# alanqrwang/nwhead

Measured on AMD Instinct MI355X. Metric: query-predictions/sec, higher is better.
Workload: dtype f32; 1 GPU; K3 predict('full'): B=256 queries/step vs bank N=50000 d=512 C=200, bank sharded 1-way, 26 query batches coalesced per launch; B=256, N_support=50000, d=512, C=200, parallelism=support-shard x1

## Files before the change

include/nwhead_hip.h:

```cpp
#ifndef NWHEAD_HIP_H
#define NWHEAD_HIP_H

#include <stddef.h>
#include <stdint.h>

#ifdef __cplusplus
extern "C" {
#endif

#define NW_ABI_VERSION 2

typedef enum {
    NW_SCORE_EUCLIDEAN = 0,
    NW_SCORE_HYPERSPHERE = 1,
    NW_SCORE_COSINE = 2,
    NW_SCORE_DOT = 3,
    NW_SCORE_CLIP = 4
} nw_score_kind;

typedef enum {
    NW_OK = 0,
    NW_ERR_INVALID_ARG = -1,
    NW_ERR_UNSUPPORTED = -2,
    NW_ERR_WORKSPACE = -3,
    NW_ERR_LAUNCH = -4,
    NW_ERR_NO_DEVICE = -5
} nw_status;

int nw_abi_version(void);
const char *nw_status_string(int status);
int nw_device_check(void);

int nw_scores_f32(const float *q, const float *s, float *scores,
                  int64_t B, int64_t N, int64_t d,
                  int kind, const float *logit_scale_dev, int sup_batched, void *stream);

int nw_row_norm2_f32(const float *x, float *n2, int64_t rows, int64_t d, void *stream);

int nw_split_rows_f16x2(const float *x, float *out_split, float *row_scale, float *row_norm2,
                        int64_t rows, int64_t d, void *stream);

typedef struct nw_fwd_opts {
    uint32_t struct_size;
    int32_t persistent_wgs;
    int32_t force_split;
    int32_t reserved;
    const void *tables;
    size_t tables_bytes;
    const int64_t *tables_sy;
    int64_t tables_N;
} nw_fwd_opts;

size_t nw_fwd_workspace_bytes(int64_t B, int64_t N, int64_t d, int64_t C);
int nw_fwd_f32(const float *q, const float *s, const int64_t *sy, const float *s_norm2,
               const float *s_split, const float *s_scale,
               float *out, float *scores_out, float *lse_out, float *weights_out,
               void *workspace, size_t workspace_bytes,
               int64_t B, int64_t N, int64_t d, int64_t C,
               int kind, const float *logit_scale_dev,
               int sup_batched, int labels_batched, const nw_fwd_opts *opts, void *stream);

int nw_fwd_partial_f32(const float *q, const float *s, const int64_t *sy, const float *s_norm2,
                       const float *s_split, const float *s_scale,
                       float *m, float *den, float *num,
                       void *workspace, size_t workspace_bytes,
                       int64_t B, int64_t N, int64_t d, int64_t C,
                       int kind, const float *logit_scale_dev, const nw_fwd_opts *opts, void *stream);
int nw_merge_finalize_f32(const float *m, const float *den, const float *num, float *out,
                          int64_t G, int64_t B, int64_t C,
                          int64_t stride_m, int64_t stride_den, int64_t stride_num,
                          const int64_t *class_lo, int64_t C_local, void *stream);

size_t nw_bank_tables_bytes(int64_t N);
int nw_bank_tables_build(const int64_t *sy, int64_t N, int64_t C, void *tables, size_t tables_bytes, void *stream);


size_t nw_bwd_workspace_bytes(int64_t B, int64_t N, int64_t d, int64_t C, int kind, int sup_batched);
int nw_bwd_f32(const float *q, const float *s, const int64_t *sy,
               const float *scores, const float *lse, const float *out, const float *gout,
               float *gq, float *gs, float *glogit_scale,
               void *workspace, size_t workspace_bytes,
               int64_t B, int64_t N, int64_t d, int64_t C,
               int kind, const float *logit_scale_dev,
               int sup_batched, int labels_batched, void *stream);
int nw_bwd_uses_split(int64_t B, int64_t N, int64_t d, int64_t C, int sup_batched);
int nw_bwd_bank_f32(const float *q, const float *s, const float *s_norm2, const float *s_split,
                    const float *s_scale, const int64_t *sy,
                    const float *scores, const float *lse, const float *out, const float *gout,
                    float *gq, float *gs, float *glogit_scale,
                    void *workspace, size_t workspace_bytes,
                    int64_t B, int64_t N, int64_t d, int64_t C,
                    int kind, const float *logit_scale_dev,
                    int sup_batched, int labels_batched, void *stream);


int nw_support_influence_f32(const float *probs, const int64_t *qy, const float *w,
                             const int64_t *sy, float *infl,
// ... 182 lines not shown
```

nwhead_amd/_lib.py:

```python
from __future__ import annotations

import ctypes as C
import os

_HERE = os.path.dirname(os.path.abspath(__file__))
LIB_PATH = os.environ.get("NW_HIP_LIB") or os.path.join(_HERE, "csrc", "libnwhead_hip.so")

SCORE_KINDS = {"euclidean": 0, "hypersphere_euclidean": 1, "cosine": 2, "dotproduct": 3, "clip": 4}

_p = C.c_void_p
_i64 = C.c_int64
_int = C.c_int
_sz = C.c_size_t

SIGNATURES = {
    "nw_abi_version": (_int, []),
    "nw_status_string": (C.c_char_p, [_int]),
    "nw_device_check": (_int, []),
    "nw_scores_f32": (_int, [_p, _p, _p, _i64, _i64, _i64, _int, _p, _int, _p]),
    "nw_fwd_workspace_bytes": (_sz, [_i64, _i64, _i64, _i64]),
    "nw_row_norm2_f32": (_int, [_p, _p, _i64, _i64, _p]),
    "nw_split_rows_f16x2": (_int, [_p, _p, _p, _p, _i64, _i64, _p]),
    "nw_fwd_f32": (_int, [_p, _p, _p, _p, _p, _p, _p, _p, _p, _p, _p, _sz, _i64, _i64, _i64, _i64, _int, _p, _int, _int, _p, _p]),
    "nw_fwd_partial_f32": (_int, [_p, _p, _p, _p, _p, _p, _p, _p, _p, _p, _sz, _i64, _i64, _i64, _i64, _int, _p, _p, _p]),
    "nw_merge_finalize_f32": (_int, [_p, _p, _p, _p, _i64, _i64, _i64, _i64, _i64, _i64, _p, _i64, _p]),
    "nw_bank_tables_bytes": (_sz, [_i64]),
    "nw_bank_tables_build": (_int, [_p, _i64, _i64, _p, _sz, _p]),
    "nw_bwd_workspace_bytes": (_sz, [_i64, _i64, _i64, _i64, _int, _int]),
    "nw_bwd_f32": (_int, [_p] * 10 + [_p, _sz, _i64, _i64, _i64, _i64, _int, _p, _int, _int, _p]),
    "nw_bwd_uses_split": (_int, [_i64, _i64, _i64, _i64, _int]),
    "nw_bwd_bank_f32": (_int, [_p] * 13 + [_p, _sz, _i64, _i64, _i64, _i64, _int, _p, _int, _int, _p]),
    "nw_support_influence_f32": (_int, [_p, _p, _p, _p, _p, _i64, _i64, _i64, _p]),
    "nw_aggregate_f32": (_int, [_p] * 5 + [_i64, _i64, _i64, _int, _p]),
    "nw_aggregate_bwd_f32": (_int, [_p] * 6 + [_i64, _i64, _i64, _int, _p]),
    "nw_fwd_influence_f32": (_int, [_p] * 11 + [_sz, _i64, _i64, _i64, _i64, _int, _p, _p, _p]),
    "nw_topk_f32": (_int, [_p, _p, _p, _i64, _i64, _i64, _p]),
    "nw_scale_shift_relu_f32": (_int, [_p, _p, _p, _p, _i64, _i64, _i64, _i64, _int, _p]),
    "nw_bias_act_nhwc_f32": (_int, [_p, _p, _p, _int, _p, _i64, _i64, _p]),
    "nw_scale_shift_relu_avgpool2_f32": (_int, [_p, _p, _p, _p, _i64, _i64, _i64, _i64, _i64, _int, _p]),
    "nw_conv3x3_workgroups": (_i64, [_i64, _i64, _i64, _i64, _i64]),
    "nw_conv3x3_workspace_bytes": (_sz, [_i64, _i64, _i64, _i64, _i64]),
    "nw_conv3x3_f32": (_int, [_p, _i64, _p, _p, _p, _i64, _int, _p, _i64, _p, _sz, _i64, _i64, _i64, _i64, _i64, _p]),
    "nw_conv1x1_workspace_bytes": (_sz, [_i64, _i64, _i64, _i64]),
    "nw_conv1x1_f32": (_int, [_p, _i64, _p, _p, _int, _p, _p, _int, _p, _i64, _p, _sz, _i64, _i64, _i64, _i64, _p]),
    "nw_bn_relu_train_fwd_f32": (_int, [_p] * 10 + [_i64, _i64, _i64, _i64, C.c_float, C.c_float, _int, _p]),
    "nw_bn_relu_train_bwd_f32": (_int, [_p] * 12 + [_i64, _i64, _i64, _i64, _i64, _int, _p]),
    "nw_absmax_f32": (_int, [_p, _i64, _p, _p]),
    "nw_to_nhwc_pad_f32": (_int, [_p, _p, _p, _i64, _i64, _i64, _i64, _i64, _i64, _i64, _p]),
    "nw_conv2d_nhwc_supported": (_int, [_i64] * 9),
    "nw_conv2d_nhwc_f16x2": (_int, [_p, _p, _p, _p, _p, _p, _int, _p, _p] + [_i64] * 11 + [_p, _p]),
# ... 64 lines not shown
        raise NWHipError("libnwhead_hip.so ABI version mismatch")
    _lib = lib
    sync_knobs()
    return lib


class WgradJob(C.Structure):
    _fields_ = [("x", C.c_void_p), ("amax_x", C.c_void_p), ("gy", C.c_void_p), ("amax_g", C.c_void_p), ("dw", C.c_void_p)] + \
               [(k, C.c_int64) for k in ("n", "H", "W", "Cin", "Cout", "KH", "KW", "stride", "pad", "ldx", "ldg", "out_oihw")] + \
               [("pre_x", C.c_void_p)] + [(k, C.c_int64) for k in ("rowrun_stride", "in_H", "in_W", "row0", "col0")]


class SgdParam(C.Structure):
    _fields_ = [("param", C.c_void_p), ("grad", C.c_void_p), ("momentum_buf", C.c_void_p), ("n", C.c_int64)]


class ConvBnStat(C.Structure):
    _fields_ = [("x", C.c_void_p), ("ldx", C.c_int64), ("mean", C.c_void_p), ("invstd", C.c_void_p), ("gamma", C.c_void_p),
                ("beta", C.c_void_p), ("partials", C.c_void_p)]


class FwdOpts(C.Structure):
    _fields_ = [("struct_size", C.c_uint32), ("persistent_wgs", C.c_int32), ("force_split", C.c_int32),
                ("reserved", C.c_int32), ("tables", C.c_void_p), ("tables_bytes", C.c_size_t),
                ("tables_sy", C.c_void_p), ("tables_N", C.c_int64)]


KNOBS = ("pvar", "qg", "tile_rs", "merge_mq", "merge_per_query", "merge_no_global_tables", "persistent_any_rs", "no_persistent",
         "split_queries", "bwd_no_mfma", "bwd_split", "coeff_threads", "xgemm_wgs", "xgemm_nbuf", "split_lbits", "conv_gather",
         "conv_max_wgs", "wgrad_min_stages", "conv_skip_cfgs", "wgrad_batch_wgs", "bn_inline_fin", "conv_moments_per_tile",
         "conv_force_cfg")
_KNOB_UNSET = -2 ** 31
_knob_state = {}


def sync_knobs():
    if _lib is None:
        return
    for k in KNOBS:
        v = os.environ.get("NW_" + k.upper())
        val = _KNOB_UNSET if v is None or v == "" else int(v)
        if _knob_state.get(k, _KNOB_UNSET) != val:
            _lib.nw_debug_set(k.encode(), val)
            _knob_state[k] = val


def force_split():
    return os.environ.get("NW_SPLIT_ALWAYS", "") == "1"


def fwd_opts(tables=None, tables_bytes=0, persistent_wgs=0, tables_sy=None, tables_n=-1):
    return FwdOpts(C.sizeof(FwdOpts), int(persistent_wgs), int(force_split()), 0, tables, int(tables_bytes), tables_sy,
                   int(tables_n))


def check(status: int, what: str):
    if status != 0:
        msg = load().nw_status_string(status).decode()
        raise NWHipError(f"{what}: {msg} (status {status})")
```

nwhead_amd/csrc/capi.hip:

```cpp
#include <cstddef>
#include <cstdlib>
#include <string.h>
#include "nw_internal.h"

namespace {
inline size_t align256(size_t x) { return (x + 255) & ~(size_t)255; }
inline bool bad_kind(int kind) { return kind < NW_SCORE_EUCLIDEAN || kind > NW_SCORE_CLIP; }
}

static bool split_pays(int64_t B, int64_t N, int64_t d) {
    return nw::fwd_opts().force_split || (double)B * (double)N * (double)d >= 2.0e8;
}

namespace nw {
namespace {
thread_local FwdOpts tl_fwd_opts;
int g_knobs[KNOB_COUNT];
bool g_knobs_init = [] { for (int& k : g_knobs) k = KNOB_UNSET; return true; }();
const char* const knob_names[KNOB_COUNT] = {
    "pvar", "qg", "tile_rs", "merge_mq", "merge_per_query", "merge_no_global_tables", "persistent_any_rs", "no_persistent",
    "split_queries", "bwd_no_mfma", "bwd_split", "coeff_threads", "xgemm_wgs", "xgemm_nbuf", "split_lbits", "conv_gather",
    "conv_max_wgs", "wgrad_min_stages", "conv_skip_cfgs", "wgrad_batch_wgs", "bn_inline_fin", "conv_moments_per_tile",
    "conv_force_cfg"};
}
const FwdOpts& fwd_opts() { return tl_fwd_opts; }
int knob(int id) { return (id >= 0 && id < KNOB_COUNT) ? __atomic_load_n(&g_knobs[id], __ATOMIC_RELAXED) : KNOB_UNSET; }
}

namespace {
struct OptsGuard {
    nw::FwdOpts saved;
    explicit OptsGuard(const nw_fwd_opts* o) : saved(nw::tl_fwd_opts) {
        nw::FwdOpts f;
        if (o && o->struct_size >= offsetof(nw_fwd_opts, tables)) {
            f.persistent_wgs = o->persistent_wgs;
            f.force_split = o->force_split;
        }
        if (o && o->struct_size >= sizeof(nw_fwd_opts)) {
            f.tables = static_cast<const char*>(o->tables);
            f.tables_bytes = o->tables_bytes;
            f.tables_sy = o->tables_sy;
            f.tables_N = o->tables_N;
        }
        nw::tl_fwd_opts = f;
    }
    ~OptsGuard() { nw::tl_fwd_opts = saved; }
};
}

extern "C" int nw_debug_set(const char* name, int value) {
    if (!name) return NW_ERR_INVALID_ARG;
    for (int k = 0; k < nw::KNOB_COUNT; ++k)
        if (!strcmp(name, nw::knob_names[k])) {
            __atomic_store_n(&nw::g_knobs[k], value, __ATOMIC_RELAXED);
            return NW_OK;
        }
    return NW_ERR_INVALID_ARG;
}

extern "C" int nw_abi_version(void) { return NW_ABI_VERSION; }

extern "C" const char* nw_status_string(int status) {
    switch (status) {
        case NW_OK: return "ok";
        case NW_ERR_INVALID_ARG: return "invalid argument";
// ... 191 lines not shown
```

nwhead_amd/csrc/fused.hip:

```cpp
#include <mutex>
#include <utility>
#include <vector>
#include "fused_impl.h"
#include <cstring>

namespace nw {

#define NW_EXTERN_FUSED_KIND(K)                                                                          \
    extern template int launch_fused_kind<K>(const float*, const float*, const int64_t*, const float*,   \
                                             const float*,                                               \
                                             const float*, float*, float*, float*, float*, float*,       \
                                             float*, void*, size_t, int, int, int, int, hipStream_t);
NW_EXTERN_FUSED_KIND(NW_SCORE_EUCLIDEAN)
NW_EXTERN_FUSED_KIND(NW_SCORE_HYPERSPHERE)
NW_EXTERN_FUSED_KIND(NW_SCORE_COSINE)
NW_EXTERN_FUSED_KIND(NW_SCORE_DOT)
NW_EXTERN_FUSED_KIND(NW_SCORE_CLIP)
#undef NW_EXTERN_FUSED_KIND

namespace {
struct TileTimer {
    bool on = false;
    std::vector<std::pair<hipEvent_t, hipEvent_t>> ev;
    std::vector<std::pair<hipEvent_t, hipEvent_t>> pool;
// ... 67 lines not shown
    for (const auto& m : map)
        if (!strcmp(m.n, name)) return knob(m.k) == 1;
    return false;
}

inline size_t al256(size_t x) { return (x + 255) & ~(size_t)255; }

size_t fused_layout(int64_t B, int64_t n_stiles, int BS, char* base, FusedWs* ws, int64_t C) {
    size_t off = 0;
    auto take = [&](size_t bytes) {
        char* p = base ? base + off : nullptr;
        off += al256(bytes);
        return p;
    };
    FusedWs w;
    w.m = reinterpret_cast<float*>(take((size_t)n_stiles * B * 4));
    w.den = reinterpret_cast<float*>(take((size_t)n_stiles * B * 4));
    w.nrun = reinterpret_cast<int*>(take((size_t)n_stiles * 4));
    w.lab = reinterpret_cast<int*>(take((size_t)n_stiles * BS * 4));
    w.num = reinterpret_cast<float*>(take((size_t)n_stiles * BS * B * 4));
    w.runid = reinterpret_cast<int*>(take(((size_t)n_stiles * BS + 64) * 4));
    w.bnd = reinterpret_cast<int*>(take((size_t)n_stiles * 2 * 4));
    w.ctab = reinterpret_cast<int*>(take((size_t)C * (3 + 4) * 4));
    if (ws) *ws = w;
    return off;
}

namespace {

constexpr int MTHREADS = 512, MENT = 4, MTPT = 16;
template <bool PARTIAL, int MQ, int TMODE>
__global__ __launch_bounds__(MTHREADS) void nw_merge_runs_kernel(
    const float* __restrict__ ws_m, const float* __restrict__ ws_den, const int* __restrict__ ws_nrun,
    const int* __restrict__ ws_lab, const float* __restrict__ ws_num, float* __restrict__ out,
    float* __restrict__ lse, float* __restrict__ m_out, float* __restrict__ den_out,
    float* __restrict__ num_out, int B, int C, int n_stiles, int BS, const int* __restrict__ ctab) {
    constexpr bool TABLES = TMODE != 0;
    constexpr bool LTAB = TMODE == 1;
    constexpr int ML = MTHREADS / MQ;
    constexpr int MNS = MQ + 1;
    constexpr int NW = MTHREADS / 64;
    constexpr float LN2 = 0.693147180559945309417f;
    static_assert(MQ <= 32 && (MQ & (MQ - 1)) == 0, "a wave holds whole groups of MQ queries");
    extern __shared__ __attribute__((aligned(16))) char smem[];
    float* red = reinterpret_cast<float*>(smem);
    float* Ms = red + 2 * NW * MQ;
    float* inv_s = Ms + MQ;
    int* lds_tab = reinterpret_cast<int*>(inv_s + MQ);
    int* cnt = TMODE == 2 ? const_cast<int*>(ctab) : lds_tab;
    int* tlo = cnt + C;
    int* thi = tlo + C;
    int* ent = thi + C;
    float* res = reinterpret_cast<float*>(lds_tab + (size_t)C * (3 + MENT));
    const int tid = threadIdx.x, bq = tid & (MQ - 1), sl = tid / MQ, wave = tid >> 6;
    const int b0 = blockIdx.x * MQ;
    const int b = min(b0 + bq, B - 1);

    const bool in_regs = n_stiles <= ML * MTPT;
    float mr[MTPT], dr[MTPT];
    float M = -INFINITY;
    if (in_regs) {
#pragma unroll
        for (int u = 0; u < MTPT; ++u) {
            const int t = sl + u * ML;
            const bool ok = t < n_stiles;
            mr[u] = ok ? ws_m[(size_t)t * B + b] : -INFINITY;
            dr[u] = ok ? ws_den[(size_t)t * B + b] : 0.f;
        }
    }
    int tnr = 0, tl3[3] = {-1, -1, -1};
    const bool one_pass_tables = LTAB && n_stiles <= MTHREADS;
    if (one_pass_tables && tid < n_stiles) {
        tnr = ws_nrun[tid];
        const int* lt = ws_lab + (size_t)tid * BS;
        tl3[0] = lt[0];
        tl3[1] = lt[1];
        tl3[2] = lt[2];
    }
    if (LTAB) {
        for (int c = tid; c < C; c += MTHREADS) {
            cnt[c] = 0;
            tlo[c] = 0x7fffffff;
            thi[c] = -1;
        }
    }
    if (in_regs) {
#pragma unroll
        for (int u = 0; u < MTPT; ++u) M = fmaxf(M, mr[u]);
    } else {
        for (int t = sl; t < n_stiles; t += ML) M = fmaxf(M, ws_m[(size_t)t * B + b]);
    }
#pragma unroll
    for (int o = 32; o >= MQ; o >>= 1) M = fmaxf(M, __shfl_xor(M, o));
    if ((tid & 63) < MQ) red[wave * MQ + bq] = M;
    __syncthreads();
    if (LTAB) {
        auto add_tile = [&](int t, int nr, const int (&l3)[3]) {
            const int* lt = ws_lab + (size_t)t * BS;
            for (int r = 0; r < nr; ++r) {
                const int y = r < 3 ? l3[r] : lt[r];
                if (y < 0) continue;
                atomicMin(&tlo[y], t);
                atomicMax(&thi[y], t);
                const int slot = atomicAdd(&cnt[y], 1);
                if (slot < MENT) ent[y * MENT + slot] = t * BS + r;
            }
        };
        if (one_pass_tables) {
            if (tid < n_stiles) add_tile(tid, tnr, tl3);
        } else {
            for (int t = tid; t < n_stiles; t += MTHREADS) {
// ... 33 lines not shown
                        if (e[j] < e[j - 1]) { const int x = e[j]; e[j] = e[j - 1]; e[j - 1] = x; }
#pragma unroll
                for (int k = 0; k < MENT; ++k)
                    if (k < n) ent[c * MENT + k] = e[k];
            }
        }
    }
    den = red[NW * MQ + bq];
#pragma unroll
    for (int k = 1; k < NW; ++k) den += red[NW * MQ + k * MQ + bq];
    if (sl == 0) inv_s[bq] = 1.f / den;
    const int nq = min(MQ, B - b0);
    if (sl == 0 && bq < nq) {
        if (PARTIAL) {
            m_out[b] = M * LN2;
            den_out[b] = den;
        } else if (lse) {
            lse[b] = M * LN2 + logf(den);
        }
    }
    __syncthreads();
    int P = 1;
    while (P < 64 && 2 * P * C * MQ <= MTHREADS) P <<= 1;
    for (int xx = tid; xx < C * MQ * P; xx += MTHREADS) {
        const int x = xx / P, sub = xx - x * P;
        const int c = x / MQ, q = x - c * MQ;
        const int bb = min(b0 + q, B - 1);
        const float Mq = Ms[q];
        float acc = 0.f;
        const int n = TABLES ? cnt[c] : MENT + 1;
        if (n <= MENT) {
            int e[MENT];
            float v[MENT], mt[MENT];
#pragma unroll
            for (int k = 0; k < MENT; ++k) e[k] = ent[c * MENT + (k < n ? k : 0)];
#pragma unroll
            for (int k = 0; k < MENT; ++k) {
                if (k < n) {
                    v[k] = ws_num[(size_t)e[k] * B + bb];
                    mt[k] = ws_m[(size_t)(e[k] / BS) * B + bb];
                }
            }
#pragma unroll
            for (int k = 0; k < MENT; ++k)
                if (k < n) acc += v[k] * __builtin_amdgcn_exp2f(mt[k] - Mq);
        } else {
            const int t0 = TABLES ? tlo[c] : 0, t1 = TABLES ? thi[c] : n_stiles - 1;
            for (int t = t0 + sub; t <= t1; t += P) {
                const int nr = ws_nrun[t];
                const float f = __builtin_amdgcn_exp2f(ws_m[(size_t)t * B + bb] - Mq);
                const int* lt = ws_lab + (size_t)t * BS;
                for (int r = 0; r < nr; ++r)
                    if (lt[r] == c) acc += ws_num[((size_t)t * BS + r) * B + bb] * f;
            }
        }
        if (P > 1) {
            if (n <= MENT && sub != 0) acc = 0.f;
            for (int o = P >> 1; o > 0; o >>= 1) acc += __shfl_xor(acc, o);
            if (sub != 0) continue;
        }
        if (LTAB && MQ > 1) {
            res[c * MNS + q] = acc;
        } else if (q < nq) {
            if (PARTIAL) num_out[(size_t)bb * C + c] = acc;
            else out[(size_t)bb * C + c] = logf(acc * inv_s[q] + NW_LOG_EPS);
        }
    }
    if (!LTAB || MQ == 1) return;
    __syncthreads();
    for (int x = tid; x < nq * C; x += MTHREADS) {
        const int qq = x / C, c = x - qq * C;
        if (PARTIAL) num_out[(size_t)(b0 + qq) * C + c] = res[c * MNS + qq];
        else out[(size_t)(b0 + qq) * C + c] = logf(res[c * MNS + qq] * inv_s[qq] + NW_LOG_EPS);
    }
}

__global__ __launch_bounds__(1024) void nw_class_tables_kernel(const int* __restrict__ ws_nrun, const int* __restrict__ ws_lab,
                                                                int n_stiles, int BS, int C, int* __restrict__ ctab) {
    int* cnt = ctab;
    int* tlo = cnt + C;
    int* thi = tlo + C;
    int* ent = thi + C;
    const int tid = threadIdx.x;
    for (int c = tid; c < C; c += 1024) {
        cnt[c] = 0;
        tlo[c] = 0x7fffffff;
        thi[c] = -1;
    }
    __threadfence();
    __syncthreads();
    for (int t = tid; t < n_stiles; t += 1024) {
// ... 8 lines not shown
            if (slot < MENT) ent[y * MENT + slot] = t * BS + r;
        }
    }
    __threadfence();
    __syncthreads();
    for (int c = tid; c < C; c += 1024) {
        const int n = cnt[c];
        if (n > 1 && n <= MENT) {
            int e[MENT];
#pragma unroll
            for (int k = 0; k < MENT; ++k) e[k] = k < n ? ent[c * MENT + k] : 0x7fffffff;
#pragma unroll
            for (int i = 1; i < MENT; ++i)
#pragma unroll
                for (int j = MENT - 1; j >= i; --j)
                    if (e[j] < e[j - 1]) { const int x = e[j]; e[j] = e[j - 1]; e[j - 1] = x; }
#pragma unroll
            for (int k = 0; k < MENT; ++k)
                if (k < n) ent[c * MENT + k] = e[k];
        }
    }
}

__global__ __launch_bounds__(64) void nw_run_tables_kernel(const int64_t* __restrict__ sy, int N, int C, int BS,
                                                           int* __restrict__ runid, int* __restrict__ nrun,
                                                           int* __restrict__ lab_out, int* __restrict__ bnd) {
    const int st = blockIdx.x, lane = threadIdx.x, s0 = st * BS;
    if (lane < 2) bnd[2 * st + lane] = BS;
    __syncthreads();
    int lab[3], flag[3];
#pragma unroll
    for (int u = 0; u < 3; ++u) {
        const int t = 3 * lane + u, j = s0 + t;
        int64_t y = -1;
        if (t < BS && j < N) y = sy[j];
        lab[u] = ((uint64_t)y < (uint64_t)C) ? (int)y : -1;
    }
    const int prev_last = __shfl_up(lab[2], 1);
    flag[0] = (lane == 0) || (lab[0] != prev_last);
    flag[1] = lab[1] != lab[0];
    flag[2] = lab[2] != lab[1];
    int incl = flag[0] + flag[1] + flag[2];
#pragma unroll
    for (int o = 1; o < 64; o <<= 1) {
        const int v = __shfl_up(incl, o);
        if (lane >= o) incl += v;
// ... 18 lines not shown
}

}

int split_queries_into_workspace(const float* q, void* workspace, size_t workspace_bytes, int64_t B, int64_t N, int64_t d,
                                 int64_t C, float** rows, float** scale, float** norm2, hipStream_t st) {
    const size_t total = nw_fwd_workspace_bytes(B, N, d, C);
    if (!workspace || workspace_bytes < total) return NW_ERR_WORKSPACE;
    const size_t a = al256((size_t)B * (size_t)d * sizeof(float)), b = al256((size_t)B * sizeof(float));
    char* base = static_cast<char*>(workspace) + (total - a - 3 * b);
    *rows = reinterpret_cast<float*>(base);
    *scale = reinterpret_cast<float*>(base + a);
    *norm2 = reinterpret_cast<float*>(base + a + b);
    return launch_split_rows(q, *rows, *scale, *norm2, B, d, st);
}

int launch_run_tables(const FusedWs& ws, const int64_t* sy, int N, int C, int n_stiles, int BS, hipStream_t st) {
    if (BS > 192) return NW_ERR_UNSUPPORTED;
    hipLaunchKernelGGL(nw_run_tables_kernel, dim3(n_stiles), dim3(64), 0, st, sy, N, C, BS, ws.runid, ws.nrun, ws.lab, ws.bnd);
    NW_CHECK_LAUNCH();
    return NW_OK;
}

constexpr int BANK_BS = 128;

size_t bank_tables_layout(int64_t n_stiles, char* base, FusedWs* ws) {
    size_t off = 0;
    auto take = [&](size_t bytes) {
        char* p = base ? base + off : nullptr;
        off += al256(bytes);
        return p;
    };
    int* nrun = reinterpret_cast<int*>(take((size_t)n_stiles * 4));
    int* lab = reinterpret_cast<int*>(take((size_t)n_stiles * BANK_BS * 4));
    int* runid = reinterpret_cast<int*>(take(((size_t)n_stiles * BANK_BS + 64) * 4));
    int* bnd = reinterpret_cast<int*>(take((size_t)n_stiles * 2 * 4));
    if (ws) {
        ws->nrun = nrun;
        ws->lab = lab;
        ws->runid = runid;
        ws->bnd = bnd;
    }
    return off;
}

bool bank_tables_take(const int64_t* sy, int N, int C, int n_stiles, int BS, FusedWs* ws) {
    (void)C;
    const FwdOpts& o = fwd_opts();
    if (!o.tables || BS != BANK_BS) return false;
    if (o.tables_sy != sy || o.tables_N != (int64_t)N) return false;
    if (o.tables_bytes < bank_tables_layout(n_stiles, nullptr, nullptr)) return false;
    bank_tables_layout(n_stiles, const_cast<char*>(o.tables), ws);
    return true;
}

int launch_merge_runs(const FusedWs& ws, float* out, float* lse, float* m, float* den, float* num,
                      int B, int C, int n_stiles, int BS, hipStream_t st) {
    auto lds_bytes = [&](int mq, bool tables) {
        return ((size_t)2 * (MTHREADS / 64) * mq + 2 * mq + (tables ? (size_t)C * (3 + MENT + mq + 1) : 0)) * sizeof(float);
    };
    const size_t cap = 150 * 1024;
    int mq = 1;
    const int force_mq = knob(KNOB_MERGE_MQ) == KNOB_UNSET ? 0 : knob(KNOB_MERGE_MQ);
    if (force_mq == 1 || force_mq == 16 || force_mq == 32) {
        mq = force_mq;
        if (lds_bytes(mq, true) > cap) mq = 1;
    } else if (B >= 512 && !env_flag("NW_MERGE_PER_QUERY")) {
        mq = n_stiles >= 128 ? 16 : 32;
        if (lds_bytes(mq, true) > cap) mq = 16;
        if (lds_bytes(mq, true) > cap) mq = 1;
    }
    const bool tables = lds_bytes(mq, true) <= cap;
    const size_t lds = lds_bytes(mq, tables);
    const int grid = (B + mq - 1) / mq;
#define NW_MERGE(P_, Q_, T_)                                                                                       \
    hipLaunchKernelGGL((nw_merge_runs_kernel<P_, Q_, T_>), dim3(grid), dim3(MTHREADS), lds, st, ws.m, ws.den, ws.nrun, \
                       ws.lab, ws.num, out, lse, m, den, num, B, C, n_stiles, BS, ws.ctab)
    if (!tables) {
        if (ws.ctab && !env_flag("NW_MERGE_NO_GLOBAL_TABLES")) {
            hipLaunchKernelGGL(nw_class_tables_kernel, dim3(1), dim3(1024), 0, st, ws.nrun, ws.lab, n_stiles, BS, C, ws.ctab);
            if (out) NW_MERGE(false, 1, 2); else NW_MERGE(true, 1, 2);
        } else {
            if (out) NW_MERGE(false, 1, 0); else NW_MERGE(true, 1, 0);
        }
    } else if (mq == 1) {
        if (out) NW_MERGE(false, 1, 1); else NW_MERGE(true, 1, 1);
    } else if (mq == 16) {
        if (out) NW_MERGE(false, 16, 1); else NW_MERGE(true, 16, 1);
    } else {
        if (out) NW_MERGE(false, 32, 1); else NW_MERGE(true, 32, 1);
    }
#undef NW_MERGE
    NW_CHECK_LAUNCH();
    return NW_OK;
}

int pick_rs(int64_t B, int64_t N, int64_t d, bool f16) {
    const int forced = env_rs();
    if (forced == 2 || forced == 4 || forced == 5 || forced == 6 || forced == 8 || forced == 10 || forced == 12)
        return forced;
    const int64_t nq = (B + BQ - 1) / BQ;
    if (forced == 0 && !f16 && d % BK == 0 && nq * ((N + 79) / 80) >= 480) return 5;
// ... 50 lines not shown
        default: return NW_ERR_UNSUPPORTED;
    }
#undef NW_KIND_CASE
}

}

extern "C" size_t nw_bank_tables_bytes(int64_t N) {
    if (N <= 0 || N > 0x7fffffffLL) return 0;
    return nw::bank_tables_layout((N + nw::BANK_BS - 1) / nw::BANK_BS, nullptr, nullptr);
}

extern "C" int nw_bank_tables_build(const int64_t* sy, int64_t N, int64_t C, void* tables, size_t tables_bytes,
                                    void* stream) {
    using namespace nw;
    if (N < 0 || C < 0 || N > 0x7fffffffLL || C > 0x7fffffffLL) return NW_ERR_INVALID_ARG;
    if (N == 0) return NW_OK;
    if (!sy || !tables || (reinterpret_cast<uintptr_t>(tables) & 15)) return NW_ERR_INVALID_ARG;
    const int64_t n_stiles = (N + BANK_BS - 1) / BANK_BS;
    FusedWs ws;
    if (tables_bytes < bank_tables_layout(n_stiles, static_cast<char*>(tables), &ws)) return NW_ERR_WORKSPACE;
    return launch_run_tables(ws, sy, (int)N, (int)C, (int)n_stiles, BANK_BS, static_cast<hipStream_t>(stream));
}
```

nwhead_amd/csrc/fused_impl.h:

```cpp
#pragma once
#include <type_traits>
#include "tile_core.h"
#include "tile_dma.h"
#include "tile_f16.h"

namespace nw {

constexpr int RUN_CAP = 192;

struct FusedWs {
    float* m;
    float* den;
    int* nrun;
    int* lab;
    float* num;
    int* runid;
    int* bnd;
    int* ctab;
};
size_t fused_layout(int64_t B, int64_t n_stiles, int BS, char* base, FusedWs* ws, int64_t C = 0);
int launch_run_tables(const FusedWs& ws, const int64_t* sy, int N, int C, int n_stiles, int BS, hipStream_t st);
bool bank_tables_take(const int64_t* sy, int N, int C, int n_stiles, int BS, FusedWs* ws);
int launch_merge_runs(const FusedWs& ws, float* out, float* lse, float* m, float* den, float* num,
                      int B, int C, int n_stiles, int BS, hipStream_t st);
int split_queries_into_workspace(const float* q, void* workspace, size_t workspace_bytes, int64_t B, int64_t N, int64_t d,
                                 int64_t C, float** rows, float** scale, float** norm2, hipStream_t st);
int device_cu_count();
bool env_flag(const char* name);
int tile_timer_start(hipStream_t st);
void tile_timer_stop(int slot, hipStream_t st);
int persistent_qgroup();
int persistent_variant();

namespace {

enum { MODE_REG = 0, MODE_DMA = 1, MODE_DMA_SN = 2, MODE_F16 = 3, MODE_F16Q = 4 };
constexpr bool mode_is_f16(int m) { return m == MODE_F16 || m == MODE_F16Q; }

template <int BS>
__device__ __forceinline__ void run_scan_wave(const int (&lab)[3], int lane, int* runid, int* runlab, int* nrun_s) {
    int flag[3];
// ... 433 lines not shown
```

nwhead_amd/csrc/nw_internal.h:

```cpp
#pragma once
#include <hip/hip_runtime.h>
#include <stdint.h>
#include "../../include/nwhead_hip.h"

#define NW_LOG_EPS 1e-12f
#define NW_NORM_EPS 1e-12f

#define NW_CHECK_LAUNCH()                          \
    do {                                           \
        if (hipGetLastError() != hipSuccess) return NW_ERR_LAUNCH; \
    } while (0)

namespace nw {

int launch_scores(const float* q, const float* s, float* scores, int64_t B, int64_t N, int64_t d,
                  int kind, const float* logit_scale_dev, int sup_batched, hipStream_t st);

int aggregate_slices(int64_t B, int64_t N);
int launch_aggregate(const float* scores, const int64_t* sy, int labels_batched, float* out,
                     float* lse, float* weights, float* m, float* den, float* num, int64_t B,
                     int64_t N, int64_t C, hipStream_t st, float* slice_ws = nullptr, size_t slice_ws_floats = 0);

int launch_merge(const float* m, const float* den, const float* num, float* out, int64_t G,
                 int64_t B, int64_t C, int64_t sm, int64_t sd, int64_t sn, const int64_t* class_lo,
// ... 10 lines not shown
};
constexpr size_t XGEMM_TAIL_BYTES = 512;
XgemmPlan xgemm_plan(int64_t M, int64_t Nn, int64_t K);
struct XgemmReduce {
    const float* part;
    const float* fac;
    const float* gfac;
    const float* rowscale;
    const float* Xo;
    float* out;
    int64_t M, Nn;
    int nchunks, fac_inverse, blocks;
};
int launch_xgemm(bool x_km, const float* X, int64_t ldx, int64_t x_rows, const float* Y, int64_t ldy, int64_t y_rows,
                 float* part, const float* fac, int fac_inverse, const float* gfac, const float* rowscale,
                 const float* Xo, float* out, int64_t M, int64_t Nn, int64_t K, hipStream_t st,
                 XgemmReduce* defer = nullptr, const XgemmReduce* pending = nullptr);

struct FwdOpts {
    const char* tables = nullptr;
    size_t tables_bytes = 0;
    const int64_t* tables_sy = nullptr;
    int64_t tables_N = -1;
    int persistent_wgs = 0;
    int force_split = 0;
};
const FwdOpts& fwd_opts();
constexpr int KNOB_UNSET = -2147483647 - 1;
enum Knob { KNOB_PVAR, KNOB_QG, KNOB_TILE_RS, KNOB_MERGE_MQ, KNOB_MERGE_PER_QUERY, KNOB_MERGE_NO_GLOBAL_TABLES,
            KNOB_PERSISTENT_ANY_RS, KNOB_NO_PERSISTENT, KNOB_SPLIT_QUERIES, KNOB_BWD_NO_MFMA, KNOB_BWD_SPLIT,
            KNOB_COEFF_THREADS, KNOB_XGEMM_WGS, KNOB_XGEMM_NBUF, KNOB_SPLIT_LBITS, KNOB_CONV_GATHER, KNOB_CONV_MAX_WGS,
            KNOB_WGRAD_MIN_STAGES, KNOB_CONV_SKIP_CFGS, KNOB_WGRAD_BATCH_WGS, KNOB_BN_INLINE_FIN, KNOB_CONV_MOMENTS_PER_TILE,
            KNOB_CONV_FORCE_CFG, KNOB_COUNT };
int knob(int id);

int launch_topk(const float* scores, int64_t* idx, float* vals, int64_t B, int64_t N, int64_t k, hipStream_t st);
int tile_timer_enable(bool on);
int tile_timer_read(double* total_us, int64_t* launches);
int pick_rs(int64_t B, int64_t N, int64_t d, bool f16 = false);
bool fused_eligible(const float* q, const float* s, int64_t B, int64_t N, int64_t d, int64_t C);
size_t fused_workspace_bytes(int64_t B, int64_t N, int64_t d, int64_t C = 0);
int launch_split_rows(const float* x, float* out, float* scale, float* norm2, int64_t rows, int64_t d,
                      hipStream_t st);
int launch_fused(const float* q, const float* s, const int64_t* sy, const float* s_norm2,
                 const float* s_scale,
                 const float* logit_scale_dev, float* out, float* scores, float* lse, float* m,
// ... 129 lines not shown
```

nwhead_amd/ops.py:

```python
from __future__ import annotations

import ctypes
import os

import torch
from torch.autograd.function import once_differentiable

from . import _lib
from ._lib import SCORE_KINDS, NWHipError


_raw_stream = getattr(torch._C, "_cuda_getCurrentRawStream", None)


def _stream(t: torch.Tensor):
    if _raw_stream is not None:
        idx = t.device.index
        return _raw_stream(torch.cuda.current_device() if idx is None else idx)
    return torch.cuda.current_stream(t.device).cuda_stream


class _OnDevice:
    __slots__ = ("ctx",)

# ... 179 lines not shown
        self.tables = self._tables_src = None
        self.tables_label_max = -1
        self._opts = {}
        if labels is not None and labels.dim() == 1 and self.split is not None:
            self.build_tables(self.sorted_labels if self.sorted_labels is not None else labels)

    def build_tables(self, labels):
        lib = _lib.load()
        lab = labels.detach()
        lab64 = lab if (lab.dtype == torch.int64 and lab.is_contiguous()) else lab.to(torch.int64).contiguous()
        N = self.shape[0]
        if lab64.dim() != 1 or lab64.numel() != N or N == 0 or not lab64.is_cuda:
            return
        lo, hi = (int(v) for v in torch.aminmax(lab64))
        if lo < 0:
            raise ValueError("support labels must be non-negative class indices (F.one_hot, nw.py:276, raises too)")
        self.tables_label_max = hi
        nbytes = lib.nw_bank_tables_bytes(N)
        tables = torch.empty(max(nbytes, 1), dtype=torch.uint8, device=lab64.device)
        with torch.cuda.device(lab64.device):
            _lib.check(lib.nw_bank_tables_build(_ptr(lab64), N, 0x7fffffff, _ptr(tables), nbytes, _stream(lab64)),
                       "nw_bank_tables_build")
        self.tables, self._tables_src, self._opts = tables, _sig(labels), {}

    def call_opts(self, sy, n_classes, persistent_wgs=0, sy_call=None):
        if self.tables is not None and _sig(sy) == self._tables_src:
            syc = sy if sy_call is None else sy_call
            if self.tables_label_max >= int(n_classes):
                raise ValueError(f"support label {self.tables_label_max} is outside [0, n_classes={int(n_classes)}) "
                                 "(the reference's F.one_hot, nw.py:276, raises)")
            key = (int(persistent_wgs), _lib.force_split(), syc.data_ptr(), syc.numel())
            op = self._opts.get(key)
            if op is None:
                if len(self._opts) > 64:
                    self._opts.clear()
                op = self._opts[key] = _lib.fwd_opts(self.tables.data_ptr(), self.tables.numel(), persistent_wgs,
                                                     syc.data_ptr(), syc.numel())
            return C_addr(op)
        return _default_opts(persistent_wgs)

    def matches(self, s):
        return _sig(s) == self._src


def _resolve_sorted_bank(s, sy, cache, per_position_outputs=False):
    if cache is None or cache.sorted_rows is None:
        return s, sy, cache
    same = sy is cache._labels_ref or (sy.data_ptr() == cache._labels_ref.data_ptr() and sy.shape == cache._labels_ref.shape)
    if per_position_outputs or not same:
        return s, sy, None
    return cache.sorted_rows, cache.sorted_labels, cache


def _apply_bank_padding(q, s, cache):
    if cache is None or not cache.pad:
        return q, s
    q = torch.nn.functional.pad(q, (0, cache.pad))
    if s.shape[-1] != cache.shape[1]:
        s = cache.rows
    return q, s
# ... 1369 lines not shown
```

Before: 7.818 million query-predictions/s.

## Precompute per-class merge tables with the bank and add bank merge path

Builds the per-class run tables (count, tile range, entry list) once per bank and class count, so the merge no longer rebuilds them on every call. It also adds a bank-table variant of the merge kernel that stages per-tile maxima in LDS and prefetches few-entry class numerators into registers before the reduction. The aim is to cut per-launch table construction and latency in the merge step. The cost is extra LDS and register pressure in the new kernel variant, plus cache-management complexity on the host side.

```diff
diff --git a/include/nwhead_hip.h b/include/nwhead_hip.h
--- a/include/nwhead_hip.h
+++ b/include/nwhead_hip.h
@@ -44,7 +44,7 @@
     uint32_t struct_size;
     int32_t persistent_wgs;
     int32_t force_split;
-    int32_t reserved;
+    int32_t tables_C;
     const void *tables;
     size_t tables_bytes;
     const int64_t *tables_sy;
@@ -73,6 +73,8 @@
 
 size_t nw_bank_tables_bytes(int64_t N);
 int nw_bank_tables_build(const int64_t *sy, int64_t N, int64_t C, void *tables, size_t tables_bytes, void *stream);
+size_t nw_bank_class_tables_bytes(int64_t N, int64_t C);
+int nw_bank_class_tables_build(const int64_t *sy, int64_t N, int64_t C, void *tables, size_t tables_bytes, void *stream);
 
 
 size_t nw_bwd_workspace_bytes(int64_t B, int64_t N, int64_t d, int64_t C, int kind, int sup_batched);
diff --git a/nwhead_amd/_lib.py b/nwhead_amd/_lib.py
--- a/nwhead_amd/_lib.py
+++ b/nwhead_amd/_lib.py
@@ -26,6 +26,8 @@
     "nw_merge_finalize_f32": (_int, [_p, _p, _p, _p, _i64, _i64, _i64, _i64, _i64, _i64, _p, _i64, _p]),
     "nw_bank_tables_bytes": (_sz, [_i64]),
     "nw_bank_tables_build": (_int, [_p, _i64, _i64, _p, _sz, _p]),
+    "nw_bank_class_tables_bytes": (_sz, [_i64, _i64]),
+    "nw_bank_class_tables_build": (_int, [_p, _i64, _i64, _p, _sz, _p]),
     "nw_bwd_workspace_bytes": (_sz, [_i64, _i64, _i64, _i64, _int, _int]),
     "nw_bwd_f32": (_int, [_p] * 10 + [_p, _sz, _i64, _i64, _i64, _i64, _int, _p, _int, _int, _p]),
     "nw_bwd_uses_split": (_int, [_i64, _i64, _i64, _i64, _int]),
@@ -136,7 +138,7 @@
 
 class FwdOpts(C.Structure):
     _fields_ = [("struct_size", C.c_uint32), ("persistent_wgs", C.c_int32), ("force_split", C.c_int32),
-                ("reserved", C.c_int32), ("tables", C.c_void_p), ("tables_bytes", C.c_size_t),
+                ("tables_C", C.c_int32), ("tables", C.c_void_p), ("tables_bytes", C.c_size_t),
                 ("tables_sy", C.c_void_p), ("tables_N", C.c_int64)]
 
 
@@ -163,9 +165,9 @@
     return os.environ.get("NW_SPLIT_ALWAYS", "") == "1"
 
 
-def fwd_opts(tables=None, tables_bytes=0, persistent_wgs=0, tables_sy=None, tables_n=-1):
-    return FwdOpts(C.sizeof(FwdOpts), int(persistent_wgs), int(force_split()), 0, tables, int(tables_bytes), tables_sy,
-                   int(tables_n))
+def fwd_opts(tables=None, tables_bytes=0, persistent_wgs=0, tables_sy=None, tables_n=-1, tables_c=0):
+    return FwdOpts(C.sizeof(FwdOpts), int(persistent_wgs), int(force_split()), int(tables_c), tables, int(tables_bytes),
+                   tables_sy, int(tables_n))
 
 
 def check(status: int, what: str):
diff --git a/nwhead_amd/csrc/capi.hip b/nwhead_amd/csrc/capi.hip
--- a/nwhead_amd/csrc/capi.hip
+++ b/nwhead_amd/csrc/capi.hip
@@ -41,6 +41,7 @@
             f.tables_bytes = o->tables_bytes;
             f.tables_sy = o->tables_sy;
             f.tables_N = o->tables_N;
+            f.tables_C = o->tables_C;
         }
         nw::tl_fwd_opts = f;
     }
diff --git a/nwhead_amd/csrc/fused.hip b/nwhead_amd/csrc/fused.hip
--- a/nwhead_amd/csrc/fused.hip
+++ b/nwhead_amd/csrc/fused.hip
@@ -113,13 +113,17 @@
     w.runid = reinterpret_cast<int*>(take(((size_t)n_stiles * BS + 64) * 4));
     w.bnd = reinterpret_cast<int*>(take((size_t)n_stiles * 2 * 4));
     w.ctab = reinterpret_cast<int*>(take((size_t)C * (3 + 4) * 4));
+    w.bank_ctab = nullptr;
     if (ws) *ws = w;
     return off;
 }
 
+constexpr int BANK_BS = 128;
+
 namespace {
 
 constexpr int MTHREADS = 512, MENT = 4, MTPT = 16;
+constexpr int MPF = 7;
 template <bool PARTIAL, int MQ, int TMODE>
 __global__ __launch_bounds__(MTHREADS) void nw_merge_runs_kernel(
     const float* __restrict__ ws_m, const float* __restrict__ ws_den, const int* __restrict__ ws_nrun,
@@ -128,6 +132,8 @@
     float* __restrict__ num_out, int B, int C, int n_stiles, int BS, const int* __restrict__ ctab) {
     constexpr bool TABLES = TMODE != 0;
     constexpr bool LTAB = TMODE == 1;
+    constexpr bool BANK = TMODE == 3;
+    constexpr bool STAGE = (LTAB || BANK) && MQ > 1;
     constexpr int ML = MTHREADS / MQ;
     constexpr int MNS = MQ + 1;
     constexpr int NW = MTHREADS / 64;
@@ -138,15 +144,47 @@
     float* Ms = red + 2 * NW * MQ;
     float* inv_s = Ms + MQ;
     int* lds_tab = reinterpret_cast<int*>(inv_s + MQ);
-    int* cnt = TMODE == 2 ? const_cast<int*>(ctab) : lds_tab;
+    int* cnt = TMODE == 2 ? const_cast<int*>(ctab)
+               : BANK     ? lds_tab + (size_t)C * (MQ + 1) + (size_t)n_stiles * MQ
+                          : lds_tab;
     int* tlo = cnt + C;
     int* thi = tlo + C;
     int* ent = thi + C;
-    float* res = reinterpret_cast<float*>(lds_tab + (size_t)C * (3 + MENT));
+    float* res = reinterpret_cast<float*>(lds_tab + (BANK ? 0 : (size_t)C * (3 + MENT)));
+    float* mt_s = res + (size_t)C * MNS;
     const int tid = threadIdx.x, bq = tid & (MQ - 1), sl = tid / MQ, wave = tid >> 6;
     const int b0 = blockIdx.x * MQ;
     const int b = min(b0 + bq, B - 1);
 
+    float pv[BANK ? MPF : 1][MENT];
+    int pn[BANK ? MPF : 1];
+    unsigned pt[BANK ? MPF : 1][MENT / 2];
+    if constexpr (BANK) {
+        for (int i = tid; i < C * (3 + MENT); i += MTHREADS) cnt[i] = ctab[i];
+        __syncthreads();
+#pragma unroll
+        for (int i = 0; i < MPF; ++i) {
+            const int xx = tid + i * MTHREADS;
+            pn[i] = 0;
+            pt[i][0] = pt[i][1] = 0u;
+            if (xx < C * MQ) {
+                const int c = xx / MQ, q = xx - c * MQ;
+                const int bb = min(b0 + q, B - 1);
+                const int n = cnt[c];
+                pn[i] = n;
+                if (n <= MENT) {
+                    int e[MENT];
+#pragma unroll
+                    for (int k = 0; k < MENT; ++k) e[k] = ent[c * MENT + (k < n ? k : 0)];
+#pragma unroll
+                    for (int k = 0; k < MENT; ++k) {
+                        pv[i][k] = k < n ? ws_num[(size_t)e[k] * B + bb] : 0.f;
+                        pt[i][k >> 1] |= (unsigned)(e[k] / BANK_BS) << (16 * (k & 1));
+                    }
+                }
+            }
+        }
+    }
     const bool in_regs = n_stiles <= ML * MTPT;
     float mr[MTPT], dr[MTPT];
     float M = -INFINITY;
@@ -178,6 +216,11 @@
     if (in_regs) {
 #pragma unroll
         for (int u = 0; u < MTPT; ++u) M = fmaxf(M, mr[u]);
+        if constexpr (BANK) {
+#pragma unroll
+            for (int u = 0; u < MTPT; ++u)
+                if (sl + u * ML < n_stiles) mt_s[(sl + u * ML) * MQ + bq] = mr[u];
+        }
     } else {
         for (int t = sl; t < n_stiles; t += ML) M = fmaxf(M, ws_m[(size_t)t * B + b]);
     }
@@ -257,7 +300,33 @@
     __syncthreads();
     int P = 1;
     while (P < 64 && 2 * P * C * MQ <= MTHREADS) P <<= 1;
-    for (int xx = tid; xx < C * MQ * P; xx += MTHREADS) {
+    if constexpr (BANK) {
+#pragma unroll
+        for (int i = 0; i < MPF; ++i) {
+            const int xx = tid + i * MTHREADS;
+            if (xx >= C * MQ) break;
+            const int c = xx / MQ, q = xx - c * MQ;
+            const float Mq = Ms[q];
+            const int n = pn[i];
+            float acc = 0.f;
+            if (n <= MENT) {
+#pragma unroll
+                for (int k = 0; k < MENT; ++k)
+                    if (k < n) acc += pv[i][k] * __builtin_amdgcn_exp2f(mt_s[((pt[i][k >> 1] >> (16 * (k & 1))) & 0xffffu) * MQ + q] - Mq);
+            } else {
+                const int bb = min(b0 + q, B - 1);
+                for (int t = tlo[c]; t <= thi[c]; ++t) {
+                    const int nr = ws_nrun[t];
+                    const float f = __builtin_amdgcn_exp2f(mt_s[t * MQ + q] - Mq);
+                    const int* lt = ws_lab + (size_t)t * BS;
+                    for (int r = 0; r < nr; ++r)
+                        if (lt[r] == c) acc += ws_num[((size_t)t * BS + r) * B + bb] * f;
+                }
+            }
+            res[c * MNS + q] = acc;
+        }
+    }
+    for (int xx = tid + (BANK ? MPF * MTHREADS : 0); xx < C * MQ * P; xx += MTHREADS) {
         const int x = xx / P, sub = xx - x * P;
         const int c = x / MQ, q = x - c * MQ;
         const int bb = min(b0 + q, B - 1);
@@ -294,14 +363,14 @@
             for (int o = P >> 1; o > 0; o >>= 1) acc += __shfl_xor(acc, o);
             if (sub != 0) continue;
         }
-        if (LTAB && MQ > 1) {
+        if (STAGE) {
             res[c * MNS + q] = acc;
         } else if (q < nq) {
             if (PARTIAL) num_out[(size_t)bb * C + c] = acc;
             else out[(size_t)bb * C + c] = logf(acc * inv_s[q] + NW_LOG_EPS);
         }
     }
-    if (!LTAB || MQ == 1) return;
+    if (!STAGE) return;
     __syncthreads();
     for (int x = tid; x < nq * C; x += MTHREADS) {
         const int qq = x / C, c = x - qq * C;
@@ -356,6 +425,44 @@
     }
 }
 
+__global__ __launch_bounds__(256) void nw_bank_ctab_reset_kernel(int C, int* __restrict__ ctab) {
+    const int c = blockIdx.x * 256 + threadIdx.x;
+    if (c >= C) return;
+    ctab[c] = 0;
+    ctab[C + c] = 0x7fffffff;
+    ctab[2 * C + c] = -1;
+#pragma unroll
+    for (int k = 0; k < MENT; ++k) ctab[3 * C + c * MENT + k] = 0;
+}
+__global__ __launch_bounds__(256) void nw_bank_ctab_count_kernel(const int* __restrict__ nrun, const int* __restrict__ lab,
+                                                                 int n_stiles, int BS, int C, int* __restrict__ ctab) {
+    const int t = blockIdx.x * 256 + threadIdx.x;
+    if (t >= n_stiles) return;
+    const int nr = nrun[t];
+    const int* lt = lab + (size_t)t * BS;
+    for (int r = 0; r < nr; ++r) {
+        const int y = lt[r];
+        if (y < 0 || y >= C) continue;
+        atomicAdd(&ctab[y], 1);
+        atomicMin(&ctab[C + y], t);
+        atomicMax(&ctab[2 * C + y], t);
+    }
+}
+__global__ __launch_bounds__(256) void nw_bank_ctab_entries_kernel(const int* __restrict__ nrun, const int* __restrict__ lab,
+                                                                   int BS, int C, int* __restrict__ ctab) {
+    const int c = blockIdx.x * 256 + threadIdx.x;
+    if (c >= C) return;
+    const int n = ctab[c];
+    if (n < 1 || n > MENT) return;
+    int k = 0;
+    for (int t = ctab[C + c]; t <= ctab[2 * C + c]; ++t) {
+        const int nr = nrun[t];
+        const int* lt = lab + (size_t)t * BS;
+        for (int r = 0; r < nr; ++r)
+            if (lt[r] == c && k < MENT) ctab[3 * C + c * MENT + k++] = t * BS + r;
+    }
+}
+
 __global__ __launch_bounds__(64) void nw_run_tables_kernel(const int64_t* __restrict__ sy, int N, int C, int BS,
                                                            int* __restrict__ runid, int* __restrict__ nrun,
                                                            int* __restrict__ lab_out, int* __restrict__ bnd) {
@@ -420,7 +527,6 @@
     return NW_OK;
 }
 
-constexpr int BANK_BS = 128;
 
 size_t bank_tables_layout(int64_t n_stiles, char* base, FusedWs* ws) {
     size_t off = 0;
@@ -442,13 +548,19 @@
     return off;
 }
 
+size_t bank_class_tables_bytes(int64_t n_stiles, int64_t C) {
+    return bank_tables_layout(n_stiles, nullptr, nullptr) + al256((size_t)C * (3 + MENT) * 4);
+}
+
 bool bank_tables_take(const int64_t* sy, int N, int C, int n_stiles, int BS, FusedWs* ws) {
-    (void)C;
     const FwdOpts& o = fwd_opts();
     if (!o.tables || BS != BANK_BS) return false;
     if (o.tables_sy != sy || o.tables_N != (int64_t)N) return false;
-    if (o.tables_bytes < bank_tables_layout(n_stiles, nullptr, nullptr)) return false;
+    const size_t run_bytes = bank_tables_layout(n_stiles, nullptr, nullptr);
+    if (o.tables_bytes < run_bytes) return false;
     bank_tables_layout(n_stiles, const_cast<char*>(o.tables), ws);
+    if (C > 0 && o.tables_C == (int64_t)C && o.tables_bytes >= bank_class_tables_bytes(n_stiles, C))
+        ws->bank_ctab = reinterpret_cast<const int*>(o.tables + run_bytes);
     return true;
 }
 
@@ -471,11 +583,28 @@
     const bool tables = lds_bytes(mq, true) <= cap;
     const size_t lds = lds_bytes(mq, tables);
     const int grid = (B + mq - 1) / mq;
+    if (ws.bank_ctab && BS == BANK_BS && mq > 1 && n_stiles <= (MTHREADS / mq) * MTPT && 2 * C * mq > MTHREADS) {
+        const size_t lds_bank = ((size_t)2 * (MTHREADS / 64) * mq + 2 * mq + (size_t)C * (mq + 1) + (size_t)n_stiles * mq + (size_t)C * (3 + MENT)) * sizeof(float);
+        if (lds_bank <= cap) {
+#define NW_MERGE_BANK(P_, Q_)                                                                                         \
+    hipLaunchKernelGGL((nw_merge_runs_kernel<P_, Q_, 3>), dim3(grid), dim3(MTHREADS), lds_bank, st, ws.m, ws.den, ws.nrun, \
+                       ws.lab, ws.num, out, lse, m, den, num, B, C, n_stiles, BS, ws.bank_ctab)
+            if (mq == 16) { if (out) NW_MERGE_BANK(false, 16); else NW_MERGE_BANK(true, 16); }
+            else { if (out) NW_MERGE_BANK(false, 32); else NW_MERGE_BANK(true, 32); }
+#undef NW_MERGE_BANK
+            NW_CHECK_LAUNCH();
+            return NW_OK;
+        }
+    }
 #define NW_MERGE(P_, Q_, T_)                                                                                       \
     hipLaunchKernelGGL((nw_merge_runs_kernel<P_, Q_, T_>), dim3(grid), dim3(MTHREADS), lds, st, ws.m, ws.den, ws.nrun, \
-                       ws.lab, ws.num, out, lse, m, den, num, B, C, n_stiles, BS, ws.ctab)
+                       ws.lab, ws.num, out, lse, m, den, num, B, C, n_stiles, BS, ctab_arg)
+    const int* ctab_arg = ws.ctab;
     if (!tables) {
-        if (ws.ctab && !env_flag("NW_MERGE_NO_GLOBAL_TABLES")) {
+        if (ws.bank_ctab && BS == BANK_BS && !env_flag("NW_MERGE_NO_GLOBAL_TABLES")) {
+            ctab_arg = ws.bank_ctab;
+            if (out) NW_MERGE(false, 1, 2); else NW_MERGE(true, 1, 2);
+        } else if (ws.ctab && !env_flag("NW_MERGE_NO_GLOBAL_TABLES")) {
             hipLaunchKernelGGL(nw_class_tables_kernel, dim3(1), dim3(1024), 0, st, ws.nrun, ws.lab, n_stiles, BS, C, ws.ctab);
             if (out) NW_MERGE(false, 1, 2); else NW_MERGE(true, 1, 2);
         } else {
@@ -572,3 +701,30 @@
     if (tables_bytes < bank_tables_layout(n_stiles, static_cast<char*>(tables), &ws)) return NW_ERR_WORKSPACE;
     return launch_run_tables(ws, sy, (int)N, (int)C, (int)n_stiles, BANK_BS, static_cast<hipStream_t>(stream));
 }
+
+extern "C" size_t nw_bank_class_tables_bytes(int64_t N, int64_t C) {
+    if (N <= 0 || N > 0x7fffffffLL || C <= 0 || C >= (1 << 30)) return 0;
+    return nw::bank_class_tables_bytes((N + nw::BANK_BS - 1) / nw::BANK_BS, C);
+}
+
+extern "C" int nw_bank_class_tables_build(const int64_t* sy, int64_t N, int64_t C, void* tables, size_t tables_bytes,
+                                          void* stream) {
+    using namespace nw;
+    if (N < 0 || C <= 0 || N > 0x7fffffffLL || C >= (1 << 30)) return NW_ERR_INVALID_ARG;
+    if (N == 0) return NW_OK;
+    if (!sy || !tables || (reinterpret_cast<uintptr_t>(tables) & 15)) return NW_ERR_INVALID_ARG;
+    const int64_t n_stiles = (N + BANK_BS - 1) / BANK_BS;
+    if (tables_bytes < bank_class_tables_bytes(n_stiles, C)) return NW_ERR_WORKSPACE;
+    hipStream_t st = static_cast<hipStream_t>(stream);
+    FusedWs ws;
+    const size_t run_bytes = bank_tables_layout(n_stiles, static_cast<char*>(tables), &ws);
+    const int rc = launch_run_tables(ws, sy, (int)N, (int)C, (int)n_stiles, BANK_BS, st);
+    if (rc != NW_OK) return rc;
+    int* ctab = reinterpret_cast<int*>(static_cast<char*>(tables) + run_bytes);
+    const int cb = (int)((C + 255) / 256), tb = (int)((n_stiles + 255) / 256);
+    hipLaunchKernelGGL(nw_bank_ctab_reset_kernel, dim3(cb), dim3(256), 0, st, (int)C, ctab);
+    hipLaunchKernelGGL(nw_bank_ctab_count_kernel, dim3(tb), dim3(256), 0, st, ws.nrun, ws.lab, (int)n_stiles, BANK_BS, (int)C, ctab);
+    hipLaunchKernelGGL(nw_bank_ctab_entries_kernel, dim3(cb), dim3(256), 0, st, ws.nrun, ws.lab, BANK_BS, (int)C, ctab);
+    NW_CHECK_LAUNCH();
+    return NW_OK;
+}
diff --git a/nwhead_amd/csrc/fused_impl.h b/nwhead_amd/csrc/fused_impl.h
--- a/nwhead_amd/csrc/fused_impl.h
+++ b/nwhead_amd/csrc/fused_impl.h
@@ -17,6 +17,7 @@
     int* runid;
     int* bnd;
     int* ctab;
+    const int* bank_ctab;
 };
 size_t fused_layout(int64_t B, int64_t n_stiles, int BS, char* base, FusedWs* ws, int64_t C = 0);
 int launch_run_tables(const FusedWs& ws, const int64_t* sy, int N, int C, int n_stiles, int BS, hipStream_t st);
diff --git a/nwhead_amd/csrc/nw_internal.h b/nwhead_amd/csrc/nw_internal.h
--- a/nwhead_amd/csrc/nw_internal.h
+++ b/nwhead_amd/csrc/nw_internal.h
@@ -56,6 +56,7 @@
     size_t tables_bytes = 0;
     const int64_t* tables_sy = nullptr;
     int64_t tables_N = -1;
+    int64_t tables_C = 0;
     int persistent_wgs = 0;
     int force_split = 0;
 };
diff --git a/nwhead_amd/ops.py b/nwhead_amd/ops.py
--- a/nwhead_amd/ops.py
+++ b/nwhead_amd/ops.py
@@ -225,6 +225,28 @@
             _lib.check(lib.nw_bank_tables_build(_ptr(lab64), N, 0x7fffffff, _ptr(tables), nbytes, _stream(lab64)),
                        "nw_bank_tables_build")
         self.tables, self._tables_src, self._opts = tables, _sig(labels), {}
+        self._tables_lab, self._class_tables = lab64, {}
+
+    merge_tables = True
+
+    def _tables_for(self, n_classes):
+        C = int(n_classes)
+        if not self.merge_tables or C <= 0:
+            return self.tables, 0
+        t = self._class_tables.get(C)
+        if t is None:
+            lib = _lib.load()
+            lab64, N = self._tables_lab, self.shape[0]
+            nbytes = lib.nw_bank_class_tables_bytes(N, C)
+            t = torch.empty(max(nbytes, 1), dtype=torch.uint8, device=lab64.device)
+            with torch.cuda.device(lab64.device):
+                _lib.check(lib.nw_bank_class_tables_build(_ptr(lab64), N, C, _ptr(t), nbytes, _stream(lab64)),
+                           "nw_bank_class_tables_build")
+            if len(self._class_tables) > 8:
+                self._class_tables.clear()
+                self._opts.clear()
+            self._class_tables[C] = t
+        return t, C
 
     def call_opts(self, sy, n_classes, persistent_wgs=0, sy_call=None):
         if self.tables is not None and _sig(sy) == self._tables_src:
@@ -232,13 +254,14 @@
             if self.tables_label_max >= int(n_classes):
                 raise ValueError(f"support label {self.tables_label_max} is outside [0, n_classes={int(n_classes)}) "
                                  "(the reference's F.one_hot, nw.py:276, raises)")
-            key = (int(persistent_wgs), _lib.force_split(), syc.data_ptr(), syc.numel())
+            key = (int(persistent_wgs), _lib.force_split(), syc.data_ptr(), syc.numel(), int(n_classes), self.merge_tables)
             op = self._opts.get(key)
             if op is None:
                 if len(self._opts) > 64:
                     self._opts.clear()
-                op = self._opts[key] = _lib.fwd_opts(self.tables.data_ptr(), self.tables.numel(), persistent_wgs,
-                                                     syc.data_ptr(), syc.numel())
+                tables, tc = self._tables_for(n_classes)
+                op = self._opts[key] = _lib.fwd_opts(tables.data_ptr(), tables.numel(), persistent_wgs,
+                                                     syc.data_ptr(), syc.numel(), tc)
             return C_addr(op)
         return _default_opts(persistent_wgs)
 
```

Result: no change. 7.829 million query-predictions/s (median of 4 runs) (+0.1%).
